# spsquared/softbody-webgpu

Measured on AMD Instinct MI355X. Metric: particle-steps/sec, higher is better.
Workload: dtype f32

## Files before the change

### softbody-webgpu_amd/csrc/sb_api.hip

```cpp
#include <algorithm>
#include <atomic>
#include <chrono>
#include <cstdio>
#include <cstdlib>
#include <cmath>
#include <cstring>
#include <memory>
#include <mutex>
#include <new>
#include <numeric>
#include <stdexcept>
#include <unordered_map>

#include "sb_engine.h"
#include "sb_edit.h"

extern "C" sb_status sb_halo_set_layout(sb_engine *e, const uint32_t *, const uint32_t *, const uint32_t *, const uint32_t *);

static thread_local std::string g_create_error;
void sb_set_create_error(const char *msg) { g_create_error = msg ? msg : ""; }

template <typename T>
static sb_status dev_alloc(sb_engine *e, T **p, size_t n)
{
// ... 1768 lines not shown
        SB_TRY(sbr_wide_counts(e, c));
        *value = c[k == "render_wide_beams"];
    }
    else if (k == "state_half") *value = e->cur;
    else if (k == "beam_state_half") *value = e->bk.K ? e->bk.cur : 0;
    else if (k.rfind("grid_stamp_", 0) == 0) {
        const int i = atoi(key + 11);
        SB_HIP(e, hipStreamSynchronize(e->stream));
        *value = (i >= 0 && i < 40 && e->dev_err) ? e->dev_err[4 + i] : 0;
    }
    else if (k.rfind("grid_ctl_", 0) == 0) {
        const int i = atoi(key + 9);
        *value = 0;
        if (e->d_grid_ctl && i >= 0 && i < (int)(sizeof(SbGridCtl) / 4)) {
            uint32_t w = 0;
            SB_HIP(e, hipStreamSynchronize(e->stream));
            SB_HIP(e, hipMemcpy(&w, (const uint32_t *)(e->d_grid_ctl + e->grid_par) + i, 4, hipMemcpyDeviceToHost));
            *value = w;
        }
    }
    else if (k == "hybrid") *value = e->hy.K;
    else if (k == "hybrid_substep_hbm_bytes") *value = e->hy.K ? blocked_bytes_model(e, e->hy) : 0;
    else if (k == "hybrid_substeps_per_launch") *value = e->hy.K ? e->hy.k_long : 0;
    else if (k == "hybrid_pending") *value = e->hy_pending ? 1 : 0;
    else if (k == "hybrid_substeps") *value = e->hy.substeps_blocked;
    else if (k == "hybrid_launches") *value = e->hy.launches_ok;
    else if (k == "hybrid_failed") *value = e->hy.launches_failed;
    else if (k == "hybrid_validate_launches") *value = e->hy.validate_launches;
    else if (k == "halo_guard") *value = e->guard_on ? 1 : 0;
    else if (k == "halo_guard_refreshes") *value = e->guard_on ? e->guard_refreshes : 0;
    else if (k == "material_mode") *value = e->mat_mode;
    else if (k == "materials") *value = e->nmat;
    else if (k == "local_index_bits") *value = e->lbits;
    else if (sbs_info(e, key, value)) {}
    else if (sbm_info(e, key, value)) {}
    else if (sbd_info(e, key, value)) {}
    else if (sbc_info(e, key, value)) {}
    else if (sby_info(e, key, value)) {}
    else if (sbx_info(e, key, value)) {}
    else if (sbg_info(e, key, value)) {}
    else SB_FAIL(e, SB_ERR_INVALID, "sb_get_info: unknown key '%s'", key);
    return SB_OK;
}

static sb_status sb_halo_configure_impl(sb_engine *e, const uint32_t *ghost_particles, uint32_t n_gp,
                            const uint32_t *send_particles, uint32_t n_sp, const uint32_t *ghost_beams,
                            uint32_t n_gb, const uint32_t *send_beams, uint32_t n_sb)
{
    if (!e) return SB_ERR_INVALID;
    if (!e->loaded) SB_FAIL(e, SB_ERR_STATE, "sb_halo_configure before sb_write_buffers");
    if ((n_gp && !ghost_particles) || (n_sp && !send_particles) || (n_gb && !ghost_beams) || (n_sb && !send_beams))
        SB_FAIL(e, SB_ERR_INVALID, "null index list");
    SB_HIP(e, hipSetDevice(e->device));
    SB_HIP(e, hipStreamSynchronize(e->stream));
    const uint32_t maxP = e->opt.max_particles, maxB = e->opt.max_beams;
    std::vector<uint32_t> internal_of_index(maxP, 0xFFFFFFFFu), slot_of_beam(maxB, 0xFFFFFFFFu);
    for (uint32_t i = 0; i < e->P; i++) internal_of_index[e->h_pidx[i]] = i;
    for (uint32_t u = 0; u < sb_user_beams(e); u++) slot_of_beam[map_get(e, e->h_mapping.data(), (size_t)maxP + u)] = sb_user_slot(e, u);
    auto translate = [](const uint32_t *src, uint32_t n, const std::vector<uint32_t> &table, std::vector<uint32_t> &dst) {
        dst.resize(n);
        for (uint32_t k = 0; k < n; k++) {
            if (src[k] >= table.size() || table[src[k]] == 0xFFFFFFFFu) return false;
            dst[k] = table[src[k]];
        }
        return true;
    };
// ... 394 lines not shown
```

### softbody-webgpu_amd/csrc/sb_blocked.hip

```cpp
#include "sb_engine.h"

#ifndef SB_BK_WAVES
#define SB_BK_WAVES 4
#endif
#ifndef SB_BK_G
#define SB_BK_G 2
#endif

SB_DEV uint32_t sbb_tile_of_block(uint32_t b, uint32_t n)
{
    uint32_t q = n >> 3, r = n & 7, x = b & 7, k = b >> 3;
    return (x < r ? x * (q + 1) : r * (q + 1) + (x - r) * q) + k;
}

struct SbBlockedPlan {
    const uint32_t *tile_p0, *tile_h0, *halo_idx, *ring_cnt, *tile_b0, *tile_e0, *tile_s0, *ent_word, *ent_state, *lvl_cnt,
        *tile_n0, *tile_nb;
    const float *ent_length;
    const float *mat_tab;
    uint32_t ntiles, K, cap, nmat, dummy_word;
};

struct SbBlockedState {
    const float *target_r, *last_r;
    float *target_w, *last_w, *strain, *stress;
    uint32_t *broken;
    const uint32_t *plastic_r;
    uint32_t *plastic_w;
};

#define SB_BK_CAP (SB_BK_MAXP * SB_BK_T + 2u + 128u)
#define SB_BK_PAD0 (SB_BK_MAXP * SB_BK_T + 2u)
#define SB_LANDED(x) asm volatile("" : "+v"(x))
#define SB_BK_DUMMY_A (SB_BK_MAXP * SB_BK_T)
#define SB_BK_DUMMY_B (SB_BK_MAXP * SB_BK_T + 1u)
#define SB_ENT_L(t, il) (((uint32_t)(il) >> 1) * (2u * SB_BK_T) + (t) + ((t) & ~63u) + ((uint32_t)(il) & 1u) * 64u)
static_assert(SB_BK_G == 2 && SB_BK_OWNB % 2u == 0u && SB_BK_HALOB % 2u == 0u, "entry slots pair up inside their class");
#define SB_BK_ROW 8u

#ifndef SB_BK_WAVES_AUX
#define SB_BK_WAVES_AUX SB_BK_WAVES
#endif
struct SbTrack {
    const SbHybridCtl *q_in;
    SbHybridCtl *q_out;
    const float4 *slots_prev;
    float4 *slots_out, *slots_zero;
    uint32_t k_prev;
    uint32_t *broken_prev;
    uint32_t *broken_ok;
};
#define SB_HY_SLOTS 64u
template <int MAT, bool AUX, bool PLAIN, bool TRACK>
__global__ __launch_bounds__(SB_BK_T) __attribute__((amdgpu_waves_per_eu(AUX ? SB_BK_WAVES_AUX : SB_BK_WAVES, AUX ? SB_BK_WAVES_AUX : SB_BK_WAVES))) void k_substep_blocked(
    SbParticleArrays r, SbParticleArrays w, SbBlockedPlan bp, SbBlockedState bs, uint32_t k_run, const SbConsts c, SbParams prm,
    const uint32_t *__restrict__ acc_flag_r, uint32_t *acc_flag_w, SbTrack tr)
{
    float moved_sum = 0.0f;
    float track_cx = 0.0f, track_cy = 0.0f;
    bool prev_broke = false;
    uint32_t hy_wv = 0u;
    float4 hy_sl = make_float4(0.f, 0.f, 0.f, 0.f);
    if (TRACK) {
        const uint32_t lane = threadIdx.x & 63u, nw = (uint32_t)(sizeof(SbHybridCtl) / 4u);
        hy_wv = ((const uint32_t *)tr.q_in)[lane < nw ? lane : 0u];
        if (tr.slots_prev) hy_sl = tr.slots_prev[lane];
    }
    __shared__ float2 s_pos[SB_BK_CAP];
    __shared__ int s_fx[SB_BK_CAP], s_fy[SB_BK_CAP];
    extern __shared__ __attribute__((aligned(16))) float s_mat[];

    const uint32_t tile = sbb_tile_of_block(blockIdx.x, bp.ntiles), tid = threadIdx.x, K = bp.K;
    const uint32_t p0 = bp.tile_p0[tile], n_own = bp.tile_p0[tile + 1] - p0, h0 = bp.tile_h0[tile];
    const uint32_t *rc = bp.ring_cnt + (size_t)tile * (K + 1), *lc = bp.lvl_cnt + (size_t)tile * K;
    const uint32_t b0 = bp.tile_b0[tile], n_ownb = bp.tile_b0[tile + 1] - b0, e0 = bp.tile_e0[tile], s0 = bp.tile_s0[tile];
    const uint32_t np_load = rc[k_run];
    const uint32_t np_move = rc[k_run - 1];
    const uint32_t ne_load = lc[k_run - 1];
    const uint32_t lmask = (1u << SB_BK_LBITS) - 1u;

    const bool acc_r = __hip_atomic_load(&acc_flag_r[tile], __ATOMIC_RELAXED, __HIP_MEMORY_SCOPE_AGENT) != 0u;
    const bool acc_w_dirty = __hip_atomic_load(&acc_flag_w[tile], __ATOMIC_RELAXED, __HIP_MEMORY_SCOPE_AGENT) != 0u;
    const bool own_plastic = __hip_atomic_load(&bs.plastic_r[tile], __ATOMIC_RELAXED, __HIP_MEMORY_SCOPE_AGENT) != 0u;
    bool nb_acc = false, nb_plastic_lane = false;
    {
        const uint32_t n0 = bp.tile_n0[tile], nn = bp.tile_n0[tile + 1] - n0;
        for (uint32_t i = tid & 63u; i < nn; i += 64u) {
            const uint32_t nb = bp.tile_nb[n0 + i];
            nb_acc |= __hip_atomic_load(&acc_flag_r[nb], __ATOMIC_RELAXED, __HIP_MEMORY_SCOPE_AGENT) != 0u;
            nb_plastic_lane |= __hip_atomic_load(&bs.plastic_r[nb], __ATOMIC_RELAXED, __HIP_MEMORY_SCOPE_AGENT) != 0u;
        }
    }
    const bool nb_plastic = __builtin_amdgcn_ballot_w64(nb_plastic_lane) != 0ull;
    if (TRACK) {
        static_assert(sizeof(SbHybridCtl) == 44, "SbHybridCtl: eleven words, named below");
#define SB_Q_U(i) ((uint32_t)__builtin_amdgcn_readlane((int)hy_wv, (i)))
#define SB_Q_F(i) __uint_as_float(SB_Q_U(i))
        float qD = SB_Q_F(0), qCx = SB_Q_F(1), qCy = SB_Q_F(2), qcx = SB_Q_F(3), qcy = SB_Q_F(4);
        const float qskin = SB_Q_F(5);
        uint32_t qbad = SB_Q_U(6), qdone = SB_Q_U(7), qsub = SB_Q_U(8);
        const uint32_t qpad = SB_Q_U(9), qfail = SB_Q_U(10);
#undef SB_Q_F
#undef SB_Q_U
        if (qbad == 0u && tr.slots_prev) {
            float m = hy_sl.x, sx = hy_sl.y, sy = hy_sl.z;
#pragma unroll
            for (int off = 32; off > 0; off >>= 1) {
                m = fmaxf(m, __shfl_xor(m, off, 64));
                sx += __shfl_xor(sx, off, 64);
                sy += __shfl_xor(sy, off, 64);
            }
            m = __uint_as_float(__builtin_amdgcn_readfirstlane(__float_as_uint(m)));
// ... 51 lines not shown
    }
#pragma unroll
    for (int i = 0; i < SB_BK_HALOB; i++) {
        const uint32_t j = SB_ENT_L(tid, i);
        sidx[i] = bp.ent_state[j < nhe ? s0 + j : 0u];
    }
    float2 pp[SB_BK_MAXP], pv[SB_BK_MAXP], pa[SB_BK_MAXP];
#pragma unroll
    for (int i = 0; i < SB_BK_OWNP; i++) {
        const uint32_t q = tid + (uint32_t)i * SB_BK_T;
        pp[i] = r.pos[q < n_own ? p0 + q : 0u];
        pv[i] = r.vel[q < n_own ? p0 + q : 0u];
        pa[i] = make_float2(0.f, 0.f);
    }
    float tg[SB_BK_MAXB], ls[SB_BK_MAXB], ln[SB_BK_MAXB];
#pragma unroll
    for (int i = 0; i < SB_BK_OWNB; i++) {
        const uint32_t j = SB_ENT_L(tid, i);
        ls[i] = bs.last_r[j < n_ownb ? b0 + j : 0u];
    }
    uint32_t word[SB_BK_MAXB];
#pragma unroll
    for (int i = 0; i < SB_BK_MAXB; i++) {
        const uint32_t j = SB_ENT_J(i);
        const bool have = i < (int)SB_BK_OWNB ? j < n_ownb : j < ne_load;
        word[i] = bp.ent_word[have ? e0 + j : 0u];
        ln[i] = MAT == 1 ? bp.ent_length[have ? e0 + j : 0u] : 1.0f;
    }
#pragma unroll
    for (int i = 0; i < SB_BK_OWNB; i++) {
        const uint32_t j = SB_ENT_L(tid, i);
        tg[i] = bs.target_r[(own_plastic && j < n_ownb) ? b0 + j : 0u];
    }
    float *s_len = s_mat + SB_BK_ROW * bp.nmat;
#pragma unroll
    for (int i = 0; i < SB_BK_HALOP; i++) {
        const uint32_t h = tid + (uint32_t)i * SB_BK_T;
        const uint32_t at = h < nh_load ? hidx[i] : 0u;
        pp[SB_BK_OWNP + i] = r.pos[at];
        pv[SB_BK_OWNP + i] = r.vel[h < nh_move ? at : 0u];
        pa[SB_BK_OWNP + i] = make_float2(0.f, 0.f);
    }
#pragma unroll
    for (int i = 0; i < SB_BK_HALOB; i++) {
        const uint32_t j = SB_ENT_L(tid, i);
        const uint32_t at = j < nhe ? sidx[i] : 0u;
        tg[SB_BK_OWNB + i] = bs.target_r[nb_plastic ? at : 0u];
        ls[SB_BK_OWNB + i] = bs.last_r[at];
    }
    const uint32_t pad_word = (SB_BK_PAD0 + 2u * (tid & 63u)) | ((SB_BK_PAD0 + 2u * (tid & 63u) + 1u) << SB_BK_LBITS);
#pragma unroll
    for (int i = 0; i < SB_BK_MAXB; i++) {
        const uint32_t j = SB_ENT_J(i);
        const bool have = i < (int)SB_BK_OWNB ? j < n_ownb : j < ne_load;
        word[i] = have ? word[i] : pad_word;
        tg[i] = have ? tg[i] : 1.0f;
        ls[i] = have ? ls[i] : 1.0f;
        if (MAT == 1) ln[i] = have ? ln[i] : 1.0f;
    }
#pragma unroll
    for (int i = 0; i < SB_BK_MAXP; i++) {
        const uint32_t q = i < (int)SB_BK_OWNP ? tid + (uint32_t)i * SB_BK_T : n_own + tid + (uint32_t)(i - (int)SB_BK_OWNP) * SB_BK_T;
        const bool moves = i < (int)SB_BK_OWNP ? q < n_own : q < np_move;
        pv[i] = moves ? pv[i] : make_float2(0.f, 0.f);
    }
    if (acc_r) {
#pragma unroll
        for (int i = 0; i < SB_BK_OWNP; i++) {
            const uint32_t q = tid + (uint32_t)i * SB_BK_T;
            if (q < n_own) pa[i] = r.acc[p0 + q];
        }
    }
    if (__syncthreads_or(nb_acc ? 1 : 0)) {
#pragma unroll
        for (int i = 0; i < SB_BK_HALOP; i++) {
            const uint32_t h = tid + (uint32_t)i * SB_BK_T;
            if (h < nh_move) pa[SB_BK_OWNP + i] = r.acc[hidx[i]];
        }
    }
    const uint32_t q_halo = n_own + tid;
#define SB_SLOT_Q(i) ((i) < (int)SB_BK_OWNP ? tid + (uint32_t)(i) * SB_BK_T : q_halo + (uint32_t)((i) - (int)SB_BK_OWNP) * SB_BK_T)
#pragma unroll
    for (int i = 0; i < SB_BK_MAXP; i++) {
        const uint32_t q = SB_SLOT_Q(i);
        const bool have = i < (int)SB_BK_OWNP ? q < n_own : q < np_load;
        if (have) {
            s_pos[q] = pp[i];
            s_fx[q] = 0;
            s_fy[q] = 0;
        }
    }
    if (MAT == 1) {
#pragma unroll
        for (int i = 0; i < SB_BK_MAXB; i++) s_len[tid + (uint32_t)i * SB_BK_T] = ln[i];
    }
    if (tid < 65u) {
        const uint32_t a = tid == 64u ? SB_BK_DUMMY_A : SB_BK_PAD0 + 2u * tid;
        s_pos[a] = make_float2(0.f, 0.f);
        s_pos[a + 1u] = make_float2(1.f, 0.f);
        s_fx[a] = s_fy[a] = s_fx[a + 1u] = s_fy[a + 1u] = 0;
    }
    for (uint32_t i = tid; i < bp.nmat; i += SB_BK_T) {
        const float *h = bp.mat_tab + 6u * i;
        float *d = s_mat + SB_BK_ROW * i;
        d[0] = h[0];
        d[1] = h[5];
        d[2] = h[1] * 65536.0f;
        d[3] = h[2] * 65536.0f;
        d[4] = h[3];
        d[5] = h[3] * h[0];
        d[6] = h[0] * h[4];
        d[7] = h[4];
    }
    uint32_t brk = 0u;
    bool any_acc = false;
    __syncthreads();
    if (!own_plastic || !nb_plastic) {
#pragma unroll
        for (int i = 0; i < SB_BK_MAXB; i++) {
            const bool own = i < (int)SB_BK_OWNB;
            const uint32_t j = SB_ENT_J(i);
            const bool have = own ? j < n_ownb : j < ne_load;
            if (have && !(own ? own_plastic : nb_plastic))
                tg[i] = MAT == 2 ? s_mat[SB_BK_ROW * (word[i] >> (2u * SB_BK_LBITS))] : s_len[tid + (uint32_t)i * SB_BK_T];
        }
    }

    uint32_t nbl = __builtin_amdgcn_readfirstlane(lc[k_run - 1]), npr = __builtin_amdgcn_readfirstlane(rc[k_run - 1]);
#ifndef SB_BK_ABLATE
#define SB_BK_ABLATE 0
#endif
    for (uint32_t s = 1; s <= k_run && !((SB_BK_ABLATE & 16) && prm.time_step >= 0.0f); s++) {
        uint32_t nbl_next = 0u, npr_next = 0u;
        if (s < k_run) {
            nbl_next = lc[k_run - s - 1];
            npr_next = rc[k_run - s - 1];
        }
        if (AUX && s == k_run) {
            const uint32_t dump = bp.tile_b0[bp.ntiles] + tid;
#pragma unroll
            for (int i = 0; i < (int)SB_BK_OWNB; i++) {
                uint32_t j = SB_ENT_L(tid, i);
                asm volatile("" : "+v"(j));
                uint32_t wd = word[i];
                asm volatile("" : "+v"(wd));
                const uint32_t at = (j < n_ownb && wd != bp.dummy_word) ? b0 + j : dump;
                const float4 *row = (const float4 *)(s_mat + SB_BK_ROW * (wd >> (2u * SB_BK_LBITS)));
                const float2 qa = s_pos[wd & lmask], qb = s_pos[(wd >> SB_BK_LBITS) & lmask];
                const float4 r0 = row[0];
                const float yield_strain = row[1].x;
                float inv_length = r0.y;
                if (MAT != 2) {
                    const float len_i = s_len[tid + (uint32_t)i * SB_BK_T];
                    inv_length = sb_wave_all(len_i >= 0x1p-45f && len_i <= 0x1p45f) ? sb_rcp_gated(len_i) : sb_div(1.0f, len_i);
                }
                const float len = sb_beam_length(qa, qb);
                const float force_mag = (tg[i] - len) * (r0.z * 0x1p-16f) + (ls[i] - len) * (r0.w * 0x1p-16f);
                const float strain_v = (len - tg[i]) * inv_length;
                bs.stress[at] = force_mag * (1.0f / 20.0f);
                bs.strain[at] = sb_div(sb_abs(strain_v), yield_strain);
                asm volatile("" ::: "memory");
            }
        }
#pragma unroll
        for (int i0 = 0; i0 < SB_BK_MAXB; i0 += SB_BK_G) {
            const uint32_t j0 = SB_ENT_J(i0);
            if ((i0 < (int)SB_BK_OWNB ? j0 < n_ownb : j0 < nbl) && !((SB_BK_ABLATE & 1) && prm.time_step >= 0.0f)) {
                float2 qa[SB_BK_G], qb[SB_BK_G];
                SbBeamMat mt[SB_BK_G];
                uint32_t la[SB_BK_G], lb[SB_BK_G];
                float t_in[SB_BK_G], l_in[SB_BK_G];
                float spring_s[SB_BK_G], damp_s[SB_BK_G];
                int32_t fa[SB_BK_G][2], fb[SB_BK_G][2];
                bool broken[SB_BK_G];
#pragma unroll
                for (int u = 0; u < SB_BK_G; u++) {
                    const int i = i0 + u;
                    asm volatile("" : "+v"(word[i]));
                    la[u] = word[i] & lmask;
                    lb[u] = (word[i] >> SB_BK_LBITS) & lmask;
                    const float4 *row = (const float4 *)(s_mat + SB_BK_ROW * (word[i] >> (2u * SB_BK_LBITS)));
                    qa[u] = s_pos[la[u]];
                    qb[u] = s_pos[lb[u]];
                    const float4 r0 = row[0], r1 = row[1];
                    mt[u].sd = sb_v2{r0.z, r0.w};
                    spring_s[u] = r0.z;
                    damp_s[u] = r0.w;
                    mt[u].yield_strain = r1.x;
                    if (MAT == 2) {
                        mt[u].length = r0.x;
                        mt[u].inv_length = r0.y;
                        mt[u].yl = r1.y;
                        mt[u].ll = r1.z;
                    } else {
                        const float len_i = s_len[tid + (uint32_t)i * SB_BK_T];
                        mt[u].length = len_i;
                        mt[u].yl = r1.x * len_i;
                        mt[u].ll = len_i * r1.w;
                    }
                    t_in[u] = tg[i];
                    l_in[u] = ls[i];
                }
                if (MAT == 1) {
                    unsigned long long odd = 0ull;
#pragma unroll
                    for (int u = 0; u < SB_BK_G; u++)
                        odd |= __builtin_amdgcn_ballot_w64(!(mt[u].length >= 0x1p-45f)) | __builtin_amdgcn_ballot_w64(!(mt[u].length <= 0x1p45f));
#pragma unroll
                    for (int u = 0; u < SB_BK_G; u++) mt[u].inv_length = odd == 0ull ? sb_rcp_gated(mt[u].length) : sb_div(1.0f, mt[u].length);
                }
                bool mirrored;
                sb_beam_group<SB_BK_G>(qa, qb, mt, t_in, l_in, fa, fb, mirrored, broken);
#pragma unroll
                for (int u = 0; u < SB_BK_G; u++) {
                    const int i = i0 + u;
                    tg[i] = t_in[u];
                    ls[i] = l_in[u];
                    if (__builtin_expect(broken[u], 0)) brk |= 1u << i;
                }
                if ((SB_BK_ABLATE & 4) && prm.time_step >= 0.0f) {
                } else if (__builtin_expect(mirrored, 1)) {
#pragma unroll
                    for (int u = 0; u < SB_BK_G; u++) {
                        __hip_atomic_fetch_sub(&s_fx[la[u]], fb[u][0], __ATOMIC_RELAXED, __HIP_MEMORY_SCOPE_WORKGROUP);
                        __hip_atomic_fetch_sub(&s_fy[la[u]], fb[u][1], __ATOMIC_RELAXED, __HIP_MEMORY_SCOPE_WORKGROUP);
                        __hip_atomic_fetch_add(&s_fx[lb[u]], fb[u][0], __ATOMIC_RELAXED, __HIP_MEMORY_SCOPE_WORKGROUP);
                        __hip_atomic_fetch_add(&s_fy[lb[u]], fb[u][1], __ATOMIC_RELAXED, __HIP_MEMORY_SCOPE_WORKGROUP);
                    }
                } else {
#pragma unroll
                    for (int u = 0; u < SB_BK_G; u++) {
                        atomicAdd(&s_fx[la[u]], fa[u][0]);
                        atomicAdd(&s_fy[la[u]], fa[u][1]);
                        atomicAdd(&s_fx[lb[u]], fb[u][0]);
                        atomicAdd(&s_fy[lb[u]], fb[u][1]);
                    }
                }
            }
        }
        if (!(SB_BK_ABLATE & 32)) __syncthreads();
        float moved_now = 0.0f;
#pragma unroll
        for (int i = 0; i < SB_BK_MAXP; i++) {
            const uint32_t q = SB_SLOT_Q(i);
            if (i < (int)SB_BK_OWNP ? q < n_own : q < npr) {
                SbParticle particle;
                particle.p = s_pos[q];
                particle.v = pv[i];
                particle.a = pa[i];
                const int fx = s_fx[q], fy = s_fy[q];
                s_fx[q] = 0;
                s_fy[q] = 0;
                const float2 p_old = particle.p;
                if (!((SB_BK_ABLATE & 2) && prm.time_step >= 0.0f)) {
                    sb_particle_integrate<PLAIN>(prm, c, particle, fx, fy);
                    if (!sb_wave_all(sb_inside_walls(prm, particle))) sb_particle_walls(prm, c, particle);
                }
                if (TRACK && i < (int)SB_BK_OWNP) {
                    const float ddx = particle.p.x - p_old.x, ddy = particle.p.y - p_old.y;
                    const float m = fmaxf(sb_abs(ddx - track_cx), sb_abs(ddy - track_cy)) * 1.4142137f;
                    moved_now = fmaxf(moved_now, m < 1.0e30f ? m : 1.0e30f);
                    if (i == 0 && tid == 0 && s == k_run) {
                        if (tile < SB_HY_SLOTS) {
                            __hip_atomic_store((uint32_t *)&tr.slots_out[tile].y, __float_as_uint(sb_abs(ddx) < 1.0e30f ? ddx : 0.0f), __ATOMIC_RELAXED, __HIP_MEMORY_SCOPE_AGENT);
                            __hip_atomic_store((uint32_t *)&tr.slots_out[tile].z, __float_as_uint(sb_abs(ddy) < 1.0e30f ? ddy : 0.0f), __ATOMIC_RELAXED, __HIP_MEMORY_SCOPE_AGENT);
                        }
                    }
                }
                s_pos[q] = particle.p;
                pv[i] = particle.v;
                pa[i] = particle.a;
            }
        }
        if (TRACK) moved_sum += moved_now;
        if (!(SB_BK_ABLATE & 32)) __syncthreads();
        nbl = __builtin_amdgcn_readfirstlane(nbl_next);
        npr = __builtin_amdgcn_readfirstlane(npr_next);
    }

    uint32_t tid_s = tid;
    asm volatile("" : "+v"(tid_s));
#pragma unroll
    for (int i = 0; i < SB_BK_OWNP; i++) {
        const uint32_t q = tid_s + (uint32_t)i * SB_BK_T;
        if (q < n_own) {
            sb_store_wt(&w.pos[p0 + q], s_pos[q]);
            sb_store_wt(&w.vel[p0 + q], pv[i]);
            const bool nz = (__float_as_uint(pa[i].x) | __float_as_uint(pa[i].y)) != 0u;
            any_acc |= nz;
            if (nz || acc_w_dirty) w.acc[p0 + q] = pa[i];
        }
    }
    bool yielded = false;
    if (!own_plastic) {
#pragma unroll
        for (int i = 0; i < SB_BK_OWNB; i++) {
            const uint32_t j = SB_ENT_L(tid_s, i);
            const float len_i = MAT == 2 ? s_mat[SB_BK_ROW * (word[i] >> (2u * SB_BK_LBITS))] : s_len[tid + (uint32_t)i * SB_BK_T];
            yielded |= j < n_ownb && word[i] != bp.dummy_word && __float_as_uint(tg[i]) != __float_as_uint(len_i);
        }
    }
    const bool plastic_w = own_plastic || __syncthreads_or(yielded ? 1 : 0) != 0;
    if (tid == 0) bs.plastic_w[tile] = plastic_w ? 1u : 0u;
#pragma unroll
    for (int i = 0; i < SB_BK_OWNB; i++) {
        const uint32_t j = SB_ENT_L(tid_s, i);
        if (j < n_ownb) {
            if (__builtin_expect(word[i] != bp.dummy_word, 1)) {
                if (plastic_w) sb_store_wt(&bs.target_w[b0 + j], tg[i]);
                sb_store_wt(&bs.last_w[b0 + j], ls[i]);
                if ((brk >> i) & 1u) {
                    atomicOr(&bs.broken[(b0 + j) >> 5], 1u << ((b0 + j) & 31u));
                    if (TRACK) __hip_atomic_store((uint32_t *)&tr.slots_out[0].w, 1u, __ATOMIC_RELAXED, __HIP_MEMORY_SCOPE_AGENT);
                }
            } else {
                float keep_t = bs.target_r[b0 + j], keep_l = bs.last_r[b0 + j];
                SB_LANDED(keep_t);
                SB_LANDED(keep_l);
                bs.target_w[b0 + j] = keep_t;
                bs.last_w[b0 + j] = keep_l;
            }
        }
    }
    const int wg_any = __syncthreads_or(any_acc ? 1 : 0);
    if (tid == 0) acc_flag_w[tile] = wg_any ? 1u : 0u;
    if (TRACK) {
        __shared__ float s_moved[SB_BK_T / 64u];
        float m = moved_sum < 1.0e30f ? moved_sum : 1.0e30f;
#pragma unroll
        for (int off = 32; off > 0; off >>= 1) m = fmaxf(m, __shfl_xor(m, off, 64));
        if ((tid & 63u) == 0u) s_moved[tid >> 6] = m;
        __syncthreads();
        if (tid == 0) {
            float b = 0.0f;
            for (uint32_t v = 0; v < SB_BK_T / 64u; v++) b = fmaxf(b, s_moved[v]);
            (void)__hip_atomic_fetch_max((uint32_t *)&tr.slots_out[tile % SB_HY_SLOTS].x, __float_as_uint(b), __ATOMIC_RELAXED, __HIP_MEMORY_SCOPE_AGENT);
        }
    }
}

__global__ __launch_bounds__(64) void k_hybrid_validate(const float4 *__restrict__ slots, uint32_t ntiles, const SbHybridCtl *q_in, SbHybridCtl *q_out,
// ... 123 lines not shown
    bool differs = false;
    for (uint32_t j = threadIdx.x; j < nb; j += 256u) {
        const uint32_t wd = ent_word[e0 + j];
        if (wd == dummy_word) continue;
        const uint32_t rest = __float_as_uint(ent_length ? ent_length[e0 + j] : mat_tab[6u * (wd >> (2u * SB_BK_LBITS))]);
        differs |= __float_as_uint(target_a[b0 + j]) != rest || __float_as_uint(target_b[b0 + j]) != rest;
    }
    const int any = __syncthreads_or(differs ? 1 : 0);
    if (threadIdx.x == 0u && !any) plastic_a[tile] = plastic_b[tile] = 0u;
}

static inline uint32_t cdiv_b(uint32_t a, uint32_t b) { return (a + b - 1) / b; }

static const float kLaunchCostUs[SB_BK_KMAX + 1] = {0.0f, 18.0f, 29.5f, 41.0f, 53.0f, 64.5f, 76.5f, 88.7f, 101.0f};
uint32_t sbk_split_call(uint32_t n, uint32_t kmax, bool fewest, uint32_t *first, uint32_t *n_first)
{
    kmax = kmax < 1u ? 1u : (kmax > SB_BK_KMAX ? SB_BK_KMAX : kmax);
    uint32_t best_L = 0;
    float best = 0.0f;
    const uint32_t L_min = (n + kmax - 1) / kmax;
    for (uint32_t L = L_min; L <= n && L <= (fewest ? L_min : L_min * 2u + 1u); L++) {
        const uint32_t hi = (n + L - 1) / L, n_hi = n - (hi - 1) * L;
        const float cost = (float)n_hi * kLaunchCostUs[hi] + (float)(L - n_hi) * kLaunchCostUs[hi - 1];
        if (!best_L || cost < best) {
            best_L = L;
            best = cost;
        }
    }
    *first = best_L ? (n + best_L - 1) / best_L : 0u;
    *n_first = best_L ? n - (*first - 1) * best_L : 0u;
    return best_L;
}

static void allow_large_lds(int device)
{
    static bool done[64] = {};
    if (device < 0 || device >= 64 || done[device]) return;
    done[device] = true;
    const int bytes = 100 * 1024;
#define SB_ALLOW(A, PL, TR) (void)hipFuncSetAttribute((const void *)k_substep_blocked<1, A, PL, TR>, hipFuncAttributeMaxDynamicSharedMemorySize, bytes)
    SB_ALLOW(false, false, false); SB_ALLOW(false, true, false); SB_ALLOW(true, false, false); SB_ALLOW(true, true, false);
    SB_ALLOW(false, false, true); SB_ALLOW(false, true, true); SB_ALLOW(true, false, true); SB_ALLOW(true, true, true);
#undef SB_ALLOW
    (void)hipGetLastError();
}

static void launch_one(sb_engine *e, SbBlockedDev &bk, uint32_t k, bool aux, bool track)
{
    SbBlockedPlan bp{bk.d_tile_p0, bk.d_tile_h0, bk.d_halo_idx, bk.d_ring_cnt, bk.d_tile_b0, bk.d_tile_e0, bk.d_tile_s0, bk.d_ent_word,
                     bk.d_ent_state, bk.d_lvl_cnt, bk.d_tile_n0, bk.d_tile_nb, bk.d_ent_length, bk.d_mat, bk.ntiles, bk.plan_K, bk.cap,
                     bk.nmat, bk.dummy_word};
    SbBlockedState bs{bk.d_target[bk.cur], bk.d_last[bk.cur], bk.d_target[bk.cur ^ 1u], bk.d_last[bk.cur ^ 1u], bk.d_strain, bk.d_stress,
                      bk.d_broken, bk.d_plastic[bk.cur], bk.d_plastic[bk.cur ^ 1u]};
    SbParticleArrays r = e->part[e->cur], w = e->part[e->cur ^ 1];
    SbTrack tr{};
    if (track) {
        float4 *slots = (float4 *)bk.d_hslots;
        const uint32_t set = bk.seq % 3u, stride = SB_HY_SLOTS;
        tr.q_in = bk.d_q + bk.qpar;
        tr.q_out = bk.d_q + (bk.qpar ^ 1u);
        tr.slots_prev = bk.run_launches ? slots + ((bk.seq + 2u) % 3u) * stride : nullptr;
        tr.slots_out = slots + set * stride;
        tr.slots_zero = slots + ((bk.seq + 1u) % 3u) * stride;
        tr.k_prev = bk.k_prev;
        tr.broken_prev = bk.d_broken_new[(bk.seq + 1u) & 1u];
        tr.broken_ok = bk.d_broken;
        bs.broken = bk.d_broken_new[bk.seq & 1u];
        bk.qpar ^= 1u;
        bk.seq = (bk.seq + 1u) % 6u;
        bk.run_launches++;
        bk.k_prev = k;
    }
#define SB_LAUNCH_B(M, A, PL, TR)                                                                                            \
    k_substep_blocked<M, A, PL, TR><<<bk.ntiles, SB_BK_T, bk.lds_bytes, e->stream>>>(r, w, bp, bs, k, e->consts, e->prm,        \
                                                                                    e->d_acc_flag[e->cur], e->d_acc_flag[e->cur ^ 1], tr)
#define SB_LAUNCH_BT(M, A, PL) do { if (track) SB_LAUNCH_B(M, A, PL, true); else SB_LAUNCH_B(M, A, PL, false); } while (0)
#define SB_LAUNCH_BA(M, PL) do { if (aux) SB_LAUNCH_BT(M, true, PL); else SB_LAUNCH_BT(M, false, PL); } while (0)
    const bool plain = e->consts.drag_exp == 2.0f && e->consts.mouse_active == 0u;
    if (bk.ntiles) {
        if (bk.mat_mode == 2) {
            if (plain) SB_LAUNCH_BA(2, true); else SB_LAUNCH_BA(2, false);
        } else {
            if (plain) SB_LAUNCH_BA(1, true); else SB_LAUNCH_BA(1, false);
        }
    }
#undef SB_LAUNCH_BA
#undef SB_LAUNCH_BT
#undef SB_LAUNCH_B
    e->cur ^= 1;
    bk.cur ^= 1u;
    e->substeps_done += k;
}

void sbk_preload_blocked(const SbBlockedDev &bk, bool tracked)
{
    hipFuncAttributes a;
#define SB_TOUCH(M, A, PL, TR) (void)hipFuncGetAttributes(&a, reinterpret_cast<const void *>(&k_substep_blocked<M, A, PL, TR>))
#define SB_TOUCH_M(M)                                      \
    do {                                                   \
        if (tracked) {                                     \
            SB_TOUCH(M, false, false, true);               \
            SB_TOUCH(M, false, true, true);                \
            SB_TOUCH(M, true, false, true);                \
            SB_TOUCH(M, true, true, true);                 \
        } else {                                           \
            SB_TOUCH(M, false, false, false);              \
            SB_TOUCH(M, false, true, false);               \
            SB_TOUCH(M, true, false, false);               \
            SB_TOUCH(M, true, true, false);                \
        }                                                  \
    } while (0)
    if (bk.mat_mode == 2) SB_TOUCH_M(2);
    else SB_TOUCH_M(1);
#undef SB_TOUCH_M
#undef SB_TOUCH
    (void)hipGetLastError();
}

void sbk_launch_blocked(sb_engine *e, uint32_t n, bool write_aux)
{
    if (e->bk.mat_mode == 1) allow_large_lds(e->device);
    uint32_t k_hi = 0, n_hi = 0;
    sbk_split_call(n, e->bk.K, e->bk.fixed_depth, &k_hi, &n_hi);
    while (n) {
        const uint32_t k = n_hi ? k_hi : k_hi - 1u;
        if (n_hi) n_hi--;
        launch_one(e, e->bk, k, write_aux && k == n, false);
        e->beams.target = e->bk.d_target[e->bk.cur];
        e->beams.last = e->bk.d_last[e->bk.cur];
        n -= k;
    }
}

void sbk_hybrid_to_blocked(sb_engine *e)
{
    SbBlockedDev &h = e->hy;
    const uint32_t B = h.nbeams;
    if (!B) return;
    if (h.synced_delete_gen != e->delete_gen) {
        k_hybrid_sync_dead<<<cdiv_b(e->nbeam, 256), 256, 0, e->stream>>>(e->beams.pair, e->beams.slot, e->nbeam, h.d_slot_e0, h.d_slot_ent,
                                                                        h.d_ent_word, h.dummy_word);
        h.synced_delete_gen = e->delete_gen;
    }
    k_hybrid_to_blocked<<<h.ntiles, 256, 0, e->stream>>>(e->beams.target, e->beams.last, h.d_copy_of_g, h.d_tile_b0, h.d_tile_e0, h.d_ent_word,
                                                         h.mat_mode == 1 ? h.d_ent_length : nullptr, h.d_mat, h.d_target[h.cur],
                                                         h.d_target[h.cur ^ 1u], h.d_last[h.cur], h.d_plastic[0], h.d_plastic[1]);
// ... 40 lines not shown
```

### softbody-webgpu_amd/csrc/sb_engine.h

```cpp
#pragma once
#include <hip/hip_runtime.h>
#include <stdint.h>

#include <cstring>
#include <new>
#include <stdexcept>
#include <string>
#include <thread>
#include <vector>

#include "../../include/softbody.h"
#include "sb_physics.h"
#include "sb_tiling.h"
#include "sb_blocking.h"
#include "sb_error.h"
#include "sb_scene_codec.h"

struct SbBeamArrays {
    uint32_t *ia, *ib;
    uint32_t *pair;
    float *length, *target, *last, *spring, *damp, *yield, *limit, *strain, *stress;
    uint32_t *slot;
};

// ... 200 lines not shown

#define SB_GUARDED(e, call)                                               \
    try {                                                                 \
        return (call);                                                    \
    } catch (const std::bad_alloc &) {                                    \
        if (e) (e)->err = "out of host memory";                           \
        return SB_ERR_OOM;                                                \
    } catch (const std::exception &ex) {                                  \
        if (e) (e)->err = std::string("internal error: ") + ex.what();    \
        return SB_ERR_INVALID;                                            \
    }

static inline bool sb_has_ranks(const sb_engine *e)
{
    return e->halo_configured || e->n_ghost_p || e->n_send_p || e->n_ghost_b || e->n_send_b || e->n_peers || e->mailbox;
}

static inline uint32_t map_isz(const sb_engine *e) { return sbc::map_item_bytes(e->opt.layout); }
static inline uint32_t map_get(const sb_engine *e, const uint8_t *m, size_t id) { return sbc::map_get(e->opt.layout, m, id); }
static inline uint32_t sb_user_beams(const sb_engine *e) { return e->h_user_slot.empty() ? e->B : (uint32_t)e->h_user_slot.size(); }
static inline uint32_t sb_user_slot(const sb_engine *e, size_t u) { return e->h_user_slot.empty() ? (uint32_t)u : e->h_user_slot[u]; }

void sbk_launch_substep(sb_engine *e, bool write_aux);
uint32_t sbk_grid_mode(const sb_engine *e);
void sbk_launch_grid_settle(sb_engine *e);
void sbk_launch_delete(sb_engine *e);
void sbk_launch_lists_min_d2(sb_engine *e);
void sbk_launch_halo_clear_ghost_flags(sb_engine *e);
void sbk_launch_halo_pack(sb_engine *e, float *dst);
void sbk_launch_halo_unpack(sb_engine *e, const float *src);
void sbk_launch_peer_exchange(sb_engine *e);
void sbk_launch_halo_guard(sb_engine *e, bool init);
void sbk_launch_blocked(sb_engine *e, uint32_t n, bool write_aux);
void sbk_preload_blocked(const SbBlockedDev &bk, bool tracked);
uint32_t sbk_split_call(uint32_t n, uint32_t kmax, bool fewest, uint32_t *first, uint32_t *n_first);
void sbk_launch_delete_blocked(sb_engine *e);
void sbk_hybrid_to_blocked(sb_engine *e);
void sbk_hybrid_to_tiled(sb_engine *e, bool aux);
void sbk_hybrid_launch(sb_engine *e, const uint32_t *ks, uint32_t count, bool aux_last);
void sbr_invalidate(sb_engine *e);
void sbr_release(sb_engine *e);
double sbr_last_build_ms(const sb_engine *e);
sb_status sbr_wide_counts(sb_engine *e, uint32_t counts[2]);
sb_status sbr_copy_table(sb_engine *e, const uint32_t **copy);
void sbs_invalidate(sb_engine *e);
void sbs_release(sb_engine *e);
void sbs_drop_checkpoint(sb_engine *e);
bool sbs_info(sb_engine *e, const char *key, uint64_t *value);
bool sbm_info(sb_engine *e, const char *key, uint64_t *value);
bool sbd_info(sb_engine *e, const char *key, uint64_t *value);
bool sbc_info(sb_engine *e, const char *key, uint64_t *value);
bool sby_info(sb_engine *e, const char *key, uint64_t *value);
bool sbx_info(sb_engine *e, const char *key, uint64_t *value);
bool sbg_info(sb_engine *e, const char *key, uint64_t *value);
sb_status sb_grid_reset_hash(sb_engine *e);
```

Baseline: 88.78 billion.

## Repack beam words to LDS byte offsets over planar position/force arrays

Replaces the interleaved float2 position and separate force arrays in shared memory with four 64-dword-aligned planes (px, py, fx, fy). For material mode 2 with at most 16 materials, each beam word is repacked once at load into pre-scaled byte offsets, so the hot loop reads LDS without shift/mask/multiply address arithmetic. The material table moves into the static shared struct and the kernel launches with no dynamic LDS. Position reads now take two loads instead of one float2 load, and a new template dimension doubles the kernel variants.

```diff
diff --git a/softbody-webgpu_amd/csrc/sb_api.hip b/softbody-webgpu_amd/csrc/sb_api.hip
--- a/softbody-webgpu_amd/csrc/sb_api.hip
+++ b/softbody-webgpu_amd/csrc/sb_api.hip
@@ -1824,6 +1824,10 @@
     else if (k == "material_mode") *value = e->mat_mode;
     else if (k == "materials") *value = e->nmat;
     else if (k == "local_index_bits") *value = e->lbits;
+    else if (k == "blocked_word_format") {
+        const SbBlockedDev &bk = e->bk.K ? e->bk : e->hy;
+        *value = bk.K ? sbk_word_format(bk) : 0;
+    }
     else if (sbs_info(e, key, value)) {}
     else if (sbm_info(e, key, value)) {}
     else if (sbd_info(e, key, value)) {}
diff --git a/softbody-webgpu_amd/csrc/sb_blocked.hip b/softbody-webgpu_amd/csrc/sb_blocked.hip
--- a/softbody-webgpu_amd/csrc/sb_blocked.hip
+++ b/softbody-webgpu_amd/csrc/sb_blocked.hip
@@ -1,4 +1,7 @@
 #include "sb_engine.h"
+#include "sb_blocked_word.h"
+
+#include <type_traits>
 
 #ifndef SB_BK_WAVES
 #define SB_BK_WAVES 4
@@ -37,6 +40,39 @@
 #define SB_ENT_L(t, il) (((uint32_t)(il) >> 1) * (2u * SB_BK_T) + (t) + ((t) & ~63u) + ((uint32_t)(il) & 1u) * 64u)
 static_assert(SB_BK_G == 2 && SB_BK_OWNB % 2u == 0u && SB_BK_HALOB % 2u == 0u, "entry slots pair up inside their class");
 #define SB_BK_ROW 8u
+static_assert(SBW_LBITS == SB_BK_LBITS && SBW_CAP == SB_BK_CAP && SBW_MAT_ROW_BYTES == 4u * SB_BK_ROW, "sb_blocked_word.h restates these");
+template <bool NARROW> struct alignas(16) SbLdsPlanes {
+    uint32_t pl[4u * SBW_PLANE];
+    float mat[NARROW ? SBW_NARROW_ROWS * SB_BK_ROW : 4u];
+    SB_DEV static uint32_t rec(uint32_t q) { return 4u * q; }
+    SB_DEV static uint32_t end_a(uint32_t w) { return sbw::a4<NARROW>(w); }
+    SB_DEV static uint32_t end_b(uint32_t w) { return sbw::b4<NARROW>(w); }
+    template <int PL> SB_DEV uint32_t *at(uint32_t h) { return (uint32_t *)((char *)pl + h + sbw::plane_bytes(PL)); }
+    SB_DEV float2 pos(uint32_t h) { return make_float2(__uint_as_float(*at<SBW_PX>(h)), __uint_as_float(*at<SBW_PY>(h))); }
+    SB_DEV void set_pos(uint32_t h, float2 p)
+    {
+        *at<SBW_PX>(h) = __float_as_uint(p.x);
+        *at<SBW_PY>(h) = __float_as_uint(p.y);
+    }
+    SB_DEV uint32_t *fx(uint32_t h) { return at<SBW_FX>(h); }
+    SB_DEV uint32_t *fy(uint32_t h) { return at<SBW_FY>(h); }
+    SB_DEV void zero_sums(uint32_t h) { *fx(h) = *fy(h) = 0u; }
+};
+static_assert(sizeof(SbLdsPlanes<true>) + 16u < (1u << 16), "a material row's two 16-byte reads are inside the 16-bit offset");
+struct alignas(16) SbLdsRecords {
+    float2 p[SB_BK_CAP];
+    uint32_t sx[SB_BK_CAP], sy[SB_BK_CAP];
+    float mat[4];
+    SB_DEV static uint32_t rec(uint32_t q) { return q; }
+    SB_DEV static uint32_t end_a(uint32_t w) { return sbw::index_a(w); }
+    SB_DEV static uint32_t end_b(uint32_t w) { return sbw::index_b(w); }
+    SB_DEV float2 pos(uint32_t h) { return p[h]; }
+    SB_DEV void set_pos(uint32_t h, float2 v) { p[h] = v; }
+    SB_DEV uint32_t *fx(uint32_t h) { return &sx[h]; }
+    SB_DEV uint32_t *fy(uint32_t h) { return &sy[h]; }
+    SB_DEV void zero_sums(uint32_t h) { sx[h] = sy[h] = 0u; }
+};
+SB_DEV float sbl_row_length(const float *mat, uint32_t row32) { return *(const float *)((const char *)mat + row32); }
 
 #ifndef SB_BK_WAVES_AUX
 #define SB_BK_WAVES_AUX SB_BK_WAVES
@@ -51,7 +87,7 @@
     uint32_t *broken_ok;
 };
 #define SB_HY_SLOTS 64u
-template <int MAT, bool AUX, bool PLAIN, bool TRACK>
+template <int MAT, bool AUX, bool PLAIN, bool TRACK, bool NARROW>
 __global__ __launch_bounds__(SB_BK_T) __attribute__((amdgpu_waves_per_eu(AUX ? SB_BK_WAVES_AUX : SB_BK_WAVES, AUX ? SB_BK_WAVES_AUX : SB_BK_WAVES))) void k_substep_blocked(
     SbParticleArrays r, SbParticleArrays w, SbBlockedPlan bp, SbBlockedState bs, uint32_t k_run, const SbConsts c, SbParams prm,
     const uint32_t *__restrict__ acc_flag_r, uint32_t *acc_flag_w, SbTrack tr)
@@ -66,9 +102,12 @@
         hy_wv = ((const uint32_t *)tr.q_in)[lane < nw ? lane : 0u];
         if (tr.slots_prev) hy_sl = tr.slots_prev[lane];
     }
-    __shared__ float2 s_pos[SB_BK_CAP];
-    __shared__ int s_fx[SB_BK_CAP], s_fy[SB_BK_CAP];
-    extern __shared__ __attribute__((aligned(16))) float s_mat[];
+    constexpr bool PLANES = !(MAT == 1 && TRACK);
+    static_assert(PLANES || !NARROW, "a narrow word's fields are byte offsets into the planes");
+    using Lds = typename std::conditional<PLANES, SbLdsPlanes<NARROW>, SbLdsRecords>::type;
+    __shared__ Lds s_lds;
+    extern __shared__ __attribute__((aligned(16))) float s_dyn[];
+    float *const s_mat = NARROW ? s_lds.mat : s_dyn;
 
     const uint32_t tile = sbb_tile_of_block(blockIdx.x, bp.ntiles), tid = threadIdx.x, K = bp.K;
     const uint32_t p0 = bp.tile_p0[tile], n_own = bp.tile_p0[tile + 1] - p0, h0 = bp.tile_h0[tile];
@@ -77,7 +116,7 @@
     const uint32_t np_load = rc[k_run];
     const uint32_t np_move = rc[k_run - 1];
     const uint32_t ne_load = lc[k_run - 1];
-    const uint32_t lmask = (1u << SB_BK_LBITS) - 1u;
+    const uint32_t dummy_held = sbw::held<NARROW>(bp.dummy_word);
 
     const bool acc_r = __hip_atomic_load(&acc_flag_r[tile], __ATOMIC_RELAXED, __HIP_MEMORY_SCOPE_AGENT) != 0u;
     const bool acc_w_dirty = __hip_atomic_load(&acc_flag_w[tile], __ATOMIC_RELAXED, __HIP_MEMORY_SCOPE_AGENT) != 0u;
@@ -195,7 +234,7 @@
         const uint32_t j = SB_ENT_L(tid, i);
         tg[i] = bs.target_r[(own_plastic && j < n_ownb) ? b0 + j : 0u];
     }
-    float *s_len = s_mat + SB_BK_ROW * bp.nmat;
+    float *s_len = s_dyn + SB_BK_ROW * bp.nmat;
 #pragma unroll
     for (int i = 0; i < SB_BK_HALOP; i++) {
         const uint32_t h = tid + (uint32_t)i * SB_BK_T;
@@ -216,7 +255,7 @@
     for (int i = 0; i < SB_BK_MAXB; i++) {
         const uint32_t j = SB_ENT_J(i);
         const bool have = i < (int)SB_BK_OWNB ? j < n_ownb : j < ne_load;
-        word[i] = have ? word[i] : pad_word;
+        word[i] = sbw::held<NARROW>(have ? word[i] : pad_word);
         tg[i] = have ? tg[i] : 1.0f;
         ls[i] = have ? ls[i] : 1.0f;
         if (MAT == 1) ln[i] = have ? ln[i] : 1.0f;
@@ -248,9 +287,8 @@
         const uint32_t q = SB_SLOT_Q(i);
         const bool have = i < (int)SB_BK_OWNP ? q < n_own : q < np_load;
         if (have) {
-            s_pos[q] = pp[i];
-            s_fx[q] = 0;
-            s_fy[q] = 0;
+            s_lds.set_pos(Lds::rec(q), pp[i]);
+            s_lds.zero_sums(Lds::rec(q));
         }
     }
     if (MAT == 1) {
@@ -259,11 +297,13 @@
     }
     if (tid < 65u) {
         const uint32_t a = tid == 64u ? SB_BK_DUMMY_A : SB_BK_PAD0 + 2u * tid;
-        s_pos[a] = make_float2(0.f, 0.f);
-        s_pos[a + 1u] = make_float2(1.f, 0.f);
-        s_fx[a] = s_fy[a] = s_fx[a + 1u] = s_fy[a + 1u] = 0;
-    }
-    for (uint32_t i = tid; i < bp.nmat; i += SB_BK_T) {
+        s_lds.set_pos(Lds::rec(a), make_float2(0.f, 0.f));
+        s_lds.set_pos(Lds::rec(a + 1u), make_float2(1.f, 0.f));
+        s_lds.zero_sums(Lds::rec(a));
+        s_lds.zero_sums(Lds::rec(a + 1u));
+    }
+    const uint32_t nrows = NARROW ? min(bp.nmat, SBW_NARROW_ROWS) : bp.nmat;
+    for (uint32_t i = tid; i < nrows; i += SB_BK_T) {
         const float *h = bp.mat_tab + 6u * i;
         float *d = s_mat + SB_BK_ROW * i;
         d[0] = h[0];
@@ -285,7 +325,7 @@
             const uint32_t j = SB_ENT_J(i);
             const bool have = own ? j < n_ownb : j < ne_load;
             if (have && !(own ? own_plastic : nb_plastic))
-                tg[i] = MAT == 2 ? s_mat[SB_BK_ROW * (word[i] >> (2u * SB_BK_LBITS))] : s_len[tid + (uint32_t)i * SB_BK_T];
+                tg[i] = MAT == 2 ? sbl_row_length(s_mat, sbw::row32<NARROW>(word[i])) : s_len[tid + (uint32_t)i * SB_BK_T];
         }
     }
 
@@ -307,9 +347,9 @@
                 asm volatile("" : "+v"(j));
                 uint32_t wd = word[i];
                 asm volatile("" : "+v"(wd));
-                const uint32_t at = (j < n_ownb && wd != bp.dummy_word) ? b0 + j : dump;
-                const float4 *row = (const float4 *)(s_mat + SB_BK_ROW * (wd >> (2u * SB_BK_LBITS)));
-                const float2 qa = s_pos[wd & lmask], qb = s_pos[(wd >> SB_BK_LBITS) & lmask];
+                const uint32_t at = (j < n_ownb && wd != dummy_held) ? b0 + j : dump;
+                const float4 *row = (const float4 *)((const char *)s_mat + sbw::row32<NARROW>(wd));
+                const float2 qa = s_lds.pos(Lds::end_a(wd)), qb = s_lds.pos(Lds::end_b(wd));
                 const float4 r0 = row[0];
                 const float yield_strain = row[1].x;
                 float inv_length = r0.y;
@@ -340,11 +380,11 @@
                 for (int u = 0; u < SB_BK_G; u++) {
                     const int i = i0 + u;
                     asm volatile("" : "+v"(word[i]));
-                    la[u] = word[i] & lmask;
-                    lb[u] = (word[i] >> SB_BK_LBITS) & lmask;
-                    const float4 *row = (const float4 *)(s_mat + SB_BK_ROW * (word[i] >> (2u * SB_BK_LBITS)));
-                    qa[u] = s_pos[la[u]];
-                    qb[u] = s_pos[lb[u]];
+                    la[u] = Lds::end_a(word[i]);
+                    lb[u] = Lds::end_b(word[i]);
+                    const float4 *row = (const float4 *)((const char *)s_mat + sbw::row32<NARROW>(word[i]));
+                    qa[u] = s_lds.pos(la[u]);
+                    qb[u] = s_lds.pos(lb[u]);
                     const float4 r0 = row[0], r1 = row[1];
                     mt[u].sd = sb_v2{r0.z, r0.w};
                     spring_s[u] = r0.z;
@@ -385,18 +425,18 @@
                 } else if (__builtin_expect(mirrored, 1)) {
 #pragma unroll
                     for (int u = 0; u < SB_BK_G; u++) {
-                        __hip_atomic_fetch_sub(&s_fx[la[u]], fb[u][0], __ATOMIC_RELAXED, __HIP_MEMORY_SCOPE_WORKGROUP);
-                        __hip_atomic_fetch_sub(&s_fy[la[u]], fb[u][1], __ATOMIC_RELAXED, __HIP_MEMORY_SCOPE_WORKGROUP);
-                        __hip_atomic_fetch_add(&s_fx[lb[u]], fb[u][0], __ATOMIC_RELAXED, __HIP_MEMORY_SCOPE_WORKGROUP);
-                        __hip_atomic_fetch_add(&s_fy[lb[u]], fb[u][1], __ATOMIC_RELAXED, __HIP_MEMORY_SCOPE_WORKGROUP);
+                        __hip_atomic_fetch_sub(s_lds.fx(la[u]), (uint32_t)fb[u][0], __ATOMIC_RELAXED, __HIP_MEMORY_SCOPE_WORKGROUP);
+                        __hip_atomic_fetch_sub(s_lds.fy(la[u]), (uint32_t)fb[u][1], __ATOMIC_RELAXED, __HIP_MEMORY_SCOPE_WORKGROUP);
+                        __hip_atomic_fetch_add(s_lds.fx(lb[u]), (uint32_t)fb[u][0], __ATOMIC_RELAXED, __HIP_MEMORY_SCOPE_WORKGROUP);
+                        __hip_atomic_fetch_add(s_lds.fy(lb[u]), (uint32_t)fb[u][1], __ATOMIC_RELAXED, __HIP_MEMORY_SCOPE_WORKGROUP);
                     }
                 } else {
 #pragma unroll
                     for (int u = 0; u < SB_BK_G; u++) {
-                        atomicAdd(&s_fx[la[u]], fa[u][0]);
-                        atomicAdd(&s_fy[la[u]], fa[u][1]);
-                        atomicAdd(&s_fx[lb[u]], fb[u][0]);
-                        atomicAdd(&s_fy[lb[u]], fb[u][1]);
+                        atomicAdd(s_lds.fx(la[u]), (uint32_t)fa[u][0]);
+                        atomicAdd(s_lds.fy(la[u]), (uint32_t)fa[u][1]);
+                        atomicAdd(s_lds.fx(lb[u]), (uint32_t)fb[u][0]);
+                        atomicAdd(s_lds.fy(lb[u]), (uint32_t)fb[u][1]);
                     }
                 }
             }
@@ -408,12 +448,11 @@
             const uint32_t q = SB_SLOT_Q(i);
             if (i < (int)SB_BK_OWNP ? q < n_own : q < npr) {
                 SbParticle particle;
-                particle.p = s_pos[q];
+                particle.p = s_lds.pos(Lds::rec(q));
                 particle.v = pv[i];
                 particle.a = pa[i];
-                const int fx = s_fx[q], fy = s_fy[q];
-                s_fx[q] = 0;
-                s_fy[q] = 0;
+                const int fx = (int)*s_lds.fx(Lds::rec(q)), fy = (int)*s_lds.fy(Lds::rec(q));
+                s_lds.zero_sums(Lds::rec(q));
                 const float2 p_old = particle.p;
                 if (!((SB_BK_ABLATE & 2) && prm.time_step >= 0.0f)) {
                     sb_particle_integrate<PLAIN>(prm, c, particle, fx, fy);
@@ -430,7 +469,7 @@
                         }
                     }
                 }
-                s_pos[q] = particle.p;
+                s_lds.set_pos(Lds::rec(q), particle.p);
                 pv[i] = particle.v;
                 pa[i] = particle.a;
             }
@@ -447,7 +486,7 @@
     for (int i = 0; i < SB_BK_OWNP; i++) {
         const uint32_t q = tid_s + (uint32_t)i * SB_BK_T;
         if (q < n_own) {
-            sb_store_wt(&w.pos[p0 + q], s_pos[q]);
+            sb_store_wt(&w.pos[p0 + q], s_lds.pos(Lds::rec(q)));
             sb_store_wt(&w.vel[p0 + q], pv[i]);
             const bool nz = (__float_as_uint(pa[i].x) | __float_as_uint(pa[i].y)) != 0u;
             any_acc |= nz;
@@ -459,8 +498,8 @@
 #pragma unroll
         for (int i = 0; i < SB_BK_OWNB; i++) {
             const uint32_t j = SB_ENT_L(tid_s, i);
-            const float len_i = MAT == 2 ? s_mat[SB_BK_ROW * (word[i] >> (2u * SB_BK_LBITS))] : s_len[tid + (uint32_t)i * SB_BK_T];
-            yielded |= j < n_ownb && word[i] != bp.dummy_word && __float_as_uint(tg[i]) != __float_as_uint(len_i);
+            const float len_i = MAT == 2 ? sbl_row_length(s_mat, sbw::row32<NARROW>(word[i])) : s_len[tid + (uint32_t)i * SB_BK_T];
+            yielded |= j < n_ownb && word[i] != dummy_held && __float_as_uint(tg[i]) != __float_as_uint(len_i);
         }
     }
     const bool plastic_w = own_plastic || __syncthreads_or(yielded ? 1 : 0) != 0;
@@ -469,7 +508,7 @@
     for (int i = 0; i < SB_BK_OWNB; i++) {
         const uint32_t j = SB_ENT_L(tid_s, i);
         if (j < n_ownb) {
-            if (__builtin_expect(word[i] != bp.dummy_word, 1)) {
+            if (__builtin_expect(word[i] != dummy_held, 1)) {
                 if (plastic_w) sb_store_wt(&bs.target_w[b0 + j], tg[i]);
                 sb_store_wt(&bs.last_w[b0 + j], ls[i]);
                 if ((brk >> i) & 1u) {
@@ -659,13 +698,18 @@
     return best_L;
 }
 
+#ifndef SB_BK_NARROW
+#define SB_BK_NARROW 1
+#endif
+uint32_t sbk_word_format(const SbBlockedDev &bk) { return (SB_BK_NARROW && bk.mat_mode == 2 && bk.nmat <= SBW_NARROW_ROWS) ? 1u : 0u; }
+
 static void allow_large_lds(int device)
 {
     static bool done[64] = {};
     if (device < 0 || device >= 64 || done[device]) return;
     done[device] = true;
     const int bytes = 100 * 1024;
-#define SB_ALLOW(A, PL, TR) (void)hipFuncSetAttribute((const void *)k_substep_blocked<1, A, PL, TR>, hipFuncAttributeMaxDynamicSharedMemorySize, bytes)
+#define SB_ALLOW(A, PL, TR) (void)hipFuncSetAttribute((const void *)k_substep_blocked<1, A, PL, TR, false>, hipFuncAttributeMaxDynamicSharedMemorySize, bytes)
     SB_ALLOW(false, false, false); SB_ALLOW(false, true, false); SB_ALLOW(true, false, false); SB_ALLOW(true, true, false);
     SB_ALLOW(false, false, true); SB_ALLOW(false, true, true); SB_ALLOW(true, false, true); SB_ALLOW(true, true, true);
 #undef SB_ALLOW
@@ -698,17 +742,19 @@
         bk.run_launches++;
         bk.k_prev = k;
     }
-#define SB_LAUNCH_B(M, A, PL, TR)                                                                                            \
-    k_substep_blocked<M, A, PL, TR><<<bk.ntiles, SB_BK_T, bk.lds_bytes, e->stream>>>(r, w, bp, bs, k, e->consts, e->prm,        \
-                                                                                    e->d_acc_flag[e->cur], e->d_acc_flag[e->cur ^ 1], tr)
-#define SB_LAUNCH_BT(M, A, PL) do { if (track) SB_LAUNCH_B(M, A, PL, true); else SB_LAUNCH_B(M, A, PL, false); } while (0)
-#define SB_LAUNCH_BA(M, PL) do { if (aux) SB_LAUNCH_BT(M, true, PL); else SB_LAUNCH_BT(M, false, PL); } while (0)
+#define SB_LAUNCH_B(M, A, PL, TR, NW)                                                                                         \
+    k_substep_blocked<M, A, PL, TR, NW><<<bk.ntiles, SB_BK_T, NW ? 0 : bk.lds_bytes, e->stream>>>(r, w, bp, bs, k, e->consts, e->prm,     \
+                                                                                        e->d_acc_flag[e->cur], e->d_acc_flag[e->cur ^ 1], tr)
+#define SB_LAUNCH_BT(M, A, PL, NW) do { if (track) SB_LAUNCH_B(M, A, PL, true, NW); else SB_LAUNCH_B(M, A, PL, false, NW); } while (0)
+#define SB_LAUNCH_BA(M, PL, NW) do { if (aux) SB_LAUNCH_BT(M, true, PL, NW); else SB_LAUNCH_BT(M, false, PL, NW); } while (0)
     const bool plain = e->consts.drag_exp == 2.0f && e->consts.mouse_active == 0u;
     if (bk.ntiles) {
-        if (bk.mat_mode == 2) {
-            if (plain) SB_LAUNCH_BA(2, true); else SB_LAUNCH_BA(2, false);
+        if (sbk_word_format(bk)) {
+            if (plain) SB_LAUNCH_BA(2, true, true); else SB_LAUNCH_BA(2, false, true);
+        } else if (bk.mat_mode == 2) {
+            if (plain) SB_LAUNCH_BA(2, true, false); else SB_LAUNCH_BA(2, false, false);
         } else {
-            if (plain) SB_LAUNCH_BA(1, true); else SB_LAUNCH_BA(1, false);
+            if (plain) SB_LAUNCH_BA(1, true, false); else SB_LAUNCH_BA(1, false, false);
         }
     }
 #undef SB_LAUNCH_BA
@@ -722,23 +768,24 @@
 void sbk_preload_blocked(const SbBlockedDev &bk, bool tracked)
 {
     hipFuncAttributes a;
-#define SB_TOUCH(M, A, PL, TR) (void)hipFuncGetAttributes(&a, reinterpret_cast<const void *>(&k_substep_blocked<M, A, PL, TR>))
-#define SB_TOUCH_M(M)                                      \
+#define SB_TOUCH(M, A, PL, TR, NW) (void)hipFuncGetAttributes(&a, reinterpret_cast<const void *>(&k_substep_blocked<M, A, PL, TR, NW>))
+#define SB_TOUCH_M(M, NW)                                  \
     do {                                                   \
         if (tracked) {                                     \
-            SB_TOUCH(M, false, false, true);               \
-            SB_TOUCH(M, false, true, true);                \
-            SB_TOUCH(M, true, false, true);                \
-            SB_TOUCH(M, true, true, true);                 \
+            SB_TOUCH(M, false, false, true, NW);           \
+            SB_TOUCH(M, false, true, true, NW);            \
+            SB_TOUCH(M, true, false, true, NW);            \
+            SB_TOUCH(M, true, true, true, NW);             \
         } else {                                           \
-            SB_TOUCH(M, false, false, false);              \
-            SB_TOUCH(M, false, true, false);               \
-            SB_TOUCH(M, true, false, false);               \
-            SB_TOUCH(M, true, true, false);                \
+            SB_TOUCH(M, false, false, false, NW);          \
+            SB_TOUCH(M, false, true, false, NW);           \
+            SB_TOUCH(M, true, false, false, NW);           \
+            SB_TOUCH(M, true, true, false, NW);            \
         }                                                  \
     } while (0)
-    if (bk.mat_mode == 2) SB_TOUCH_M(2);
-    else SB_TOUCH_M(1);
+    if (sbk_word_format(bk)) SB_TOUCH_M(2, true);
+    else if (bk.mat_mode == 2) SB_TOUCH_M(2, false);
+    else SB_TOUCH_M(1, false);
 #undef SB_TOUCH_M
 #undef SB_TOUCH
     (void)hipGetLastError();
diff --git a/softbody-webgpu_amd/csrc/sb_blocked_word.h b/softbody-webgpu_amd/csrc/sb_blocked_word.h
--- /dev/null
+++ b/softbody-webgpu_amd/csrc/sb_blocked_word.h
@@ -0,0 +1,39 @@
+#pragma once
+#include <stdint.h>
+
+#if defined(__HIPCC__) || defined(__CUDACC__)
+#define SBW_HD __host__ __device__ __forceinline__
+#else
+#define SBW_HD inline
+#endif
+
+#define SBW_LBITS 12u
+#define SBW_CAP 2690u
+#define SBW_PLANE 2752u
+#define SBW_NARROW_ROWS 16u
+#define SBW_MAT_ROW_BYTES 32u
+enum { SBW_PX = 0, SBW_PY = 1, SBW_FX = 2, SBW_FY = 3 };
+
+static_assert(SBW_PLANE % 64u == 0u && SBW_PLANE >= SBW_CAP && SBW_PLANE - SBW_CAP < 64u, "a plane: the next multiple of 64 dwords");
+static_assert(4u * (SBW_CAP - 1u) < (1u << 14), "the last padding record's byte offset fits a narrow field");
+static_assert(SBW_CAP - 1u < (1u << SBW_LBITS), "... and its index a wide one");
+static_assert(4u * (3u * SBW_PLANE) < (1u << 16), "the furthest plane is inside a DS instruction's 16-bit offset");
+static_assert(3u * (SBW_PLANE / 64u) < 256u, "... and inside the 8-bit offsets of the st64 forms");
+
+namespace sbw {
+
+constexpr uint32_t plane_bytes(uint32_t pl) { return 4u * SBW_PLANE * pl; }
+
+SBW_HD uint32_t pack_wide(uint32_t a, uint32_t b, uint32_t row) { return a | (b << SBW_LBITS) | (row << (2u * SBW_LBITS)); }
+SBW_HD uint32_t pack_narrow(uint32_t a, uint32_t b, uint32_t row) { return (a << 2) | (b << 16) | (row << 28); }
+SBW_HD uint32_t repack(uint32_t wide) { return ((wide & ((1u << SBW_LBITS) - 1u)) << 2) | ((wide << 4) & 0xFFFF0000u); }
+
+template <bool NARROW> SBW_HD uint32_t held(uint32_t wide) { return NARROW ? repack(wide) : wide; }
+SBW_HD uint32_t index_a(uint32_t wide) { return wide & ((1u << SBW_LBITS) - 1u); }
+SBW_HD uint32_t index_b(uint32_t wide) { return (wide >> SBW_LBITS) & ((1u << SBW_LBITS) - 1u); }
+template <bool NARROW> SBW_HD uint32_t a4(uint32_t w) { return NARROW ? (w & 0x3FFFu) : (index_a(w) << 2); }
+template <bool NARROW> SBW_HD uint32_t b4(uint32_t w) { return NARROW ? ((w >> 14) & 0x3FFFu) : (index_b(w) << 2); }
+template <bool NARROW> SBW_HD uint32_t row(uint32_t w) { return NARROW ? (w >> 28) : (w >> (2u * SBW_LBITS)); }
+template <bool NARROW> SBW_HD uint32_t row32(uint32_t w) { return row<NARROW>(w) * SBW_MAT_ROW_BYTES; }
+
+}
diff --git a/softbody-webgpu_amd/csrc/sb_engine.h b/softbody-webgpu_amd/csrc/sb_engine.h
--- a/softbody-webgpu_amd/csrc/sb_engine.h
+++ b/softbody-webgpu_amd/csrc/sb_engine.h
@@ -256,6 +256,7 @@
 void sbk_launch_peer_exchange(sb_engine *e);
 void sbk_launch_halo_guard(sb_engine *e, bool init);
 void sbk_launch_blocked(sb_engine *e, uint32_t n, bool write_aux);
+uint32_t sbk_word_format(const SbBlockedDev &bk);
 void sbk_preload_blocked(const SbBlockedDev &bk, bool tracked);
 uint32_t sbk_split_call(uint32_t n, uint32_t kmax, bool fewest, uint32_t *first, uint32_t *n_first);
 void sbk_launch_delete_blocked(sb_engine *e);
```

Measured after the change: 90.64 billion, median of 6. +2.1%, better.
